# Slienteagle-wyb/tdmpc

Measured on AMD Instinct MI355X. Metric: plan-steps/sec (N=512, H=5, iters=6) at 1/2/4/8 MI355X vs CPU ref, higher is better.
Workload: dtype fp32

## Files before the change

tdmpc_amd/csrc/tdmpc_kernels.hip:

```cpp
#include <hip/hip_runtime.h>
#include <hiprand/hiprand_kernel.h>

#include <math.h>
#include <stdint.h>
#include <stdio.h>
#include <stdlib.h>
#include <string.h>
#include <unistd.h>

#include <algorithm>
#include <atomic>
#include <chrono>
#include <mutex>
#include <type_traits>
#include <vector>

#include "../../include/tdmpc_hip.h"

typedef float floatx16 __attribute__((ext_vector_type(16)));

#define DEVI __device__ __forceinline__

#ifdef TDMPC_STAMPS
__device__ unsigned long long* g_stamps;
// ... 3118 lines not shown
    return a;
}

struct Ctx {
    const tdmpc_dims* d; Layout w; Work k; const float* pw; hipStream_t s;
    int B, N, P, T, H, A, M, Kx;
    int path;
    long eps_env, eps_cem_off, eps_iter, eps_term_off, eps_act_off;
    mutable int split_pend = 0, split_par = 0, split_first = 0;
    mutable float split_disc = 0.f;
    mutable RowMap split_map = {1 << 30, 0, 0};
    mutable int split_rows = 0, split_t = 0;
    int z0c_ready = 0;
    int fold_ok = 0;
    int fold_heads = 0;
    int fold_policy = 0;
};

float* Xt(const Ctx& c, int t) { return c.k.X + (size_t)t * c.k.x_stride; }
const unsigned short* x6p(const Ctx& c, int i) { return (const unsigned short*)(c.pw + c.w.x6[i]); }
enum { CK_STEP = 0, CK_PI = 1, CK_Q = 2 };
int chain_wgs_kind(int kind) {
    static int v[3] = {-2, -2, -2};
    if (v[kind] == -2) {
        static const char* names[3] = {"TDMPC_CHAIN_WGS_STEP", "TDMPC_CHAIN_WGS_PI", "TDMPC_CHAIN_WGS_Q"};
        const char* e = getenv(names[kind]);
        v[kind] = e ? atoi(e) : -1;
    }
    if (v[kind] >= 0) return v[kind];
    return kind == CK_Q ? chain_wgs() / 2 : chain_wgs();
}

bool use_chain(const Ctx& c, int rows, int nprob, int kind) {
    if (c.path == TDMPC_PATH_LAYERED || c.path == TDMPC_PATH_SPLIT || c.path == TDMPC_PATH_SPLIT_X6 || !chain_shape_ok(c.w))
        return false;
    const int th = chain_wgs_kind(kind);
    return c.path != TDMPC_PATH_AUTO || (th > 0 && (rows + 31) / 32 * nprob >= th);
}

int use_x6(const Ctx& c) {
    if (c.w.M != 512) return 0;
    static int en = -1;
    if (en < 0) {
        const char* e = getenv("TDMPC_X6");
        en = e ? atoi(e) : 3;
    }
    if (en == 2) en = 3;
    if (c.path == TDMPC_PATH_CHAIN_X6 || c.path == TDMPC_PATH_WIDE) return en == 1 || en == 3 ? en : 3;
    if (c.path == TDMPC_PATH_SPLIT_X6) return 1;
    return (c.path == TDMPC_PATH_AUTO || c.path == TDMPC_PATH_CHAIN) ? en : 0;
}

int chain_rb(const Ctx& c, int rows, int nprob) {
    if (!chain16_shape_ok(c.w) || c.path == TDMPC_PATH_CHAIN32 || c.path == TDMPC_PATH_CHAIN_X6 ||
        c.path == TDMPC_PATH_WIDE)
        return 32;
    if (c.path == TDMPC_PATH_CHAIN16) return 16;
    return (rows + 31) / 32 * nprob > num_cus() / 2 ? 32 : 16;
}

ChainArgs chain0(const Ctx& c, int rows, RowMap map, int t, int K1, int q1, int nprob) {
    ChainArgs a;
    memset(&a, 0, sizeof a);
    a.rows = rows; a.M = c.M; a.K1 = K1; a.q1 = q1; a.amap = map;
    a.k1_alg = K1 == c.Kx ? c.w.L + c.w.A : c.w.L;
    a.rb = chain_rb(c, rows, nprob);
    a.x6 = a.rb == 32 ? use_x6(c) : (use_x6(c) ? 1 : 0);
    if (a.x6 == 3 && (c.w.Ap / 4 * 32 > 512 || std::max(c.w.Lr, c.w.Ar) > 4 * 4 * 32)) a.x6 = 1;
    a.nw = a.x6 == 3 ? 4 : 8;
    a.hfl = std::max((int)rup(c.Kx, 32), c.M) * a.rb;
    a.X = Xt(c, t); a.x_ts = (long)c.Kx * 32;
    return a;
}
Opnd xop(const Ctx& c, int t, int q0) { return Opnd{Xt(c, t), (long)c.Kx * 32, q0}; }
Outp xout(const Ctx& c, int t, int q0) { return Outp{Xt(c, t), (long)c.Kx * 32, q0}; }
Opnd hop(const float* H, const Ctx& c, int q0) { return Opnd{H, (long)2 * c.M * 32, q0}; }
Outp hout(float* H, const Ctx& c, int q0) { return Outp{H, (long)2 * c.M * 32, q0}; }
Opnd wop(const Ctx& c, size_t off, int K) { return Opnd{c.pw + off, (long)K * 32, 0}; }

bool use_split(const Ctx& c, int rows) {
    const Layout& w = c.w;
    if (w.M != 512 || rows > c.k.split_rows || (size_t)split_lds_floats(w.Kx, w.M) * 4 > 64 * 1024) return false;
    if (c.path == TDMPC_PATH_SPLIT || c.path == TDMPC_PATH_SPLIT_X6) return true;
    if (c.path != TDMPC_PATH_AUTO || (int)rup(w.Kx, 16) > w.M / 2) return false;
    return !use_chain(c, rows, 2, CK_STEP);
}

bool use_split_pi(const Ctx& c, int rows) {
    const Layout& w = c.w;
    if (w.M != 512 || rows > c.k.split_rows || (size_t)split_lds_floats(w.Lp, w.M) * 4 > 64 * 1024) return false;
    if (c.path == TDMPC_PATH_SPLIT || c.path == TDMPC_PATH_SPLIT_X6) return true;
    if (c.path != TDMPC_PATH_AUTO || (int)rup(w.Lp, 16) > w.M / 2) return false;
    return !use_chain(c, rows, 1, CK_PI);
}

int split_finish(const Ctx& c, int t, int rows, RowMap map, const float* zp, const float* rp, float disc, int first,
                 int last) {
    const Layout& w = c.w;
    SplitFinishArgs f;
    memset(&f, 0, sizeof f);
    f.rows = rows; f.amap = map; f.zpart = zp; f.rpart = rp; f.prow = c.k.split_rows;
    f.n3 = w.Lr; f.L = w.L; f.Lp = w.Lp; f.b3d = c.pw + w.b3d; f.b3r = c.pw + w.b3r;
    f.Xo = Xt(c, t + 1); f.x_ts = (long)c.Kx * 32; f.out_q0 = w.Ap / 4;
    f.G = c.k.G; f.rlast = c.k.rlast; f.disc = disc; f.first = first; f.last = last;
    const long nth = (long)rows * (w.Lp / 4 + 1);
    hipLaunchKernelGGL(split_finish_kernel, dim3((unsigned)((nth + 255) / 256)), dim3(256), 0, c.s, f);
    HIPCHK(hipGetLastError());
    return 0;
}

int flush_split(const Ctx& c) {
    if (!c.split_pend) return 0;
    c.split_pend = 0;
    const int par = 1 - c.split_par;
    const size_t zs = (size_t)SPLIT_S * c.k.split_rows * std::max(c.w.Lr, c.w.Ar), rs = (size_t)SPLIT_S * c.k.split_rows;
    return split_finish(c, c.split_t, c.split_rows, c.split_map, c.k.zpart + par * zs, c.k.rpart_s + par * rs,
                        c.split_disc, c.split_first, 0);
}

int z0c_k1c(const Ctx& c) { return (int)rup(c.w.Ap, 16); }
bool z0c_eligible(const Ctx& c) {
    static const int v = [] { const char* e = getenv("TDMPC_Z0C"); return e ? atoi(e) : 1; }();
    return v && z0c_k1c(c) < (int)rup(c.Kx, 16);
}
int z0c_launch(const Ctx& c) {
    hipLaunchKernelGGL(z0c_kernel, dim3(c.B, 2, (c.M + 255) / 256), dim3(256), 0, c.s, c.pw + c.w.w1x, c.pw + c.w.b1x,
                       c.k.z0, c.Kx, c.w.Ap, c.w.Lp, z0c_k1c(c), c.M, c.k.z0c);
    HIPCHK(hipGetLastError());
    return 0;
}

unsigned long long* g_p1_stamps = nullptr;

int wide_g1(const Ctx& c, bool z0c) {
    return (int)rup(z0c ? z0c_k1c(c) : c.Kx, 32) / 32;
}
bool wide_instance(int g1, int nb3, int mode) {
#define WIDE_HAS(G1, NB3, MODE) if (g1 == G1 && nb3 == NB3 && mode == (MODE)) return true;
    WIDE_FOR_EACH(WIDE_HAS)
#undef WIDE_HAS
    return false;
}
bool use_wide(const Ctx& c, int rows, const RowMap& map, bool z0c) {
    static const int en = [] { const char* e = getenv("TDMPC_WIDE"); return e ? atoi(e) : 1; }();
    if (c.w.M != 512 || !use_x6(c) || !num_cus()) return false;
    if (c.path != TDMPC_PATH_AUTO && c.path != TDMPC_PATH_CHAIN && c.path != TDMPC_PATH_WIDE) return false;
    if (c.path != TDMPC_PATH_WIDE && !en) return false;
    if (rows % 16 || map.G % 16 || map.S % 16 || map.O % 16) return false;
    if (z0c && map.G % 128) return false;
    const int g1 = wide_g1(c, z0c), nb3 = (int)rup(c.w.L, 16) / 16, mode = g1 > 5 ? WS_XS : 0;
    if (!wide_instance(g1, nb3, mode) || (c.w.fold && !wide_instance(g1, nb3, mode | WS_OUTH))) return false;
    return c.path == TDMPC_PATH_WIDE || (rows + 127) / 128 * 2 >= num_cus();
}
bool fold_on() {
    static const int v = [] { const char* e = getenv("TDMPC_FOLD"); return e ? atoi(e) : 1; }();
    return v != 0;
}
int launch_wide(const Ctx& c, int t, int rows, RowMap map, float disc, int first, int last, bool z0c, bool fold = false) {
    const Layout& w = c.w;
    const int M = c.M;
    WideArgs a;
    memset(&a, 0, sizeof a);
    auto q6 = [&](int i) { return (const unsigned short*)(c.pw + w.x6q[i]); };
    a.g1s = (int)(rup(c.Kx, 32) / 32);
    const size_t rb1 = (size_t)(M / 16) * a.g1s * 1536;
    const bool fold_in = fold && t >= 1 && !z0c, outh = fold && (!last || c.fold_heads);
    a.p[0].X1 = q6(X6_W1X); a.p[1].X1 = q6(X6_W1X) + rb1;
    a.p[0].X2 = q6(X6_W2D); a.p[1].X2 = q6(X6_W2R);
    a.p[0].b1 = c.pw + w.b1x; a.p[1].b1 = c.pw + w.b1x + M;
    if (fold_in) {
        const unsigned short* xf = (const unsigned short*)(c.pw + w.x6qw);
        a.p[0].X1 = xf; a.p[1].X1 = xf + rb1;
        a.p[0].b1 = c.pw + w.bfw; a.p[1].b1 = c.pw + w.bfw + M;
    }
    a.p[0].b2 = c.pw + w.b2d; a.p[1].b2 = c.pw + w.b2r;
    a.p[1].w3v = c.pw + w.w3r; a.p[1].b3v = c.pw + w.b3r;
    a.X3 = q6(X6_W3D); a.b3 = c.pw + w.b3d; a.nvalid = w.L; a.nstore = w.Lp;
    a.rows = rows; a.nrb = (rows + 127) / 128; a.amap = map;
    a.X = Xt(c, t); a.x_ts = (long)c.Kx * 32;
    a.kq = (z0c ? z0c_k1c(c) : c.Kx) / 4;
    a.Xo = Xt(c, t + 1); a.out_q0 = w.Ap / 4;
    a.G = c.k.G; a.rlast = c.k.rlast; a.disc = disc; a.first = first; a.last = last;
    if (z0c) { a.z0c = c.k.z0c; a.z0_G = map.G; }
    a.stamps = g_p1_stamps;
    const int g1 = wide_g1(c, z0c), nb3 = (int)rup(w.L, 16) / 16;
    const int mode = (g1 > 5 ? WS_XS : 0) | (outh ? WS_OUTH : 0);
    const dim3 grid((unsigned)rup(a.nrb, 4) * 2), block(64 * WS_NW);
    Profiler& pf = g_prof;
    const bool prof = prof_armed() && pf.cfg == 4 + CH_STEP && (pf.rows == 0 || rows == pf.rows) && !z0c;
    if (prof) {
        if (mode) snprintf(pf.kernel, sizeof pf.kernel, "wide_step_kernel<%d, %d, %s%s%s>", g1, nb3,
                           mode & WS_XS ? "XS" : "", mode == (WS_XS | WS_OUTH) ? "|" : "", mode & WS_OUTH ? "OUTH" : "");
        else snprintf(pf.kernel, sizeof pf.kernel, "wide_step_kernel<%d, %d>", g1, nb3);
    }
    HIPCHK(prof_begin(prof, c.s));
    bool done = false;
#define WIDE_LAUNCH(G1, NB3, MODE) \
    if (!done && g1 == G1 && nb3 == NB3 && mode == (MODE)) { \
        hipLaunchKernelGGL((wide_step_kernel<G1, NB3, MODE>), grid, block, (wsm_lds<G1, MODE>()), c.s, a); \
        done = true; \
    }
    WIDE_FOR_EACH(WIDE_LAUNCH)
#undef WIDE_LAUNCH
    if (!done) { snprintf(g_err, sizeof g_err, "wide step: no instance for G1 %d NB3 %d mode %d", g1, nb3, mode); return TDMPC_E_DIMS; }
    HIPCHK(hipGetLastError());
    const double K1 = w.L + w.A;
    HIPCHK(prof_end(prof, c.s, 2.0 * rows * (2 * (K1 * M + (double)M * M) + (outh ? 0.0 : (double)M * w.L) + M)));
    return 0;
}

size_t x6_w1_rows_stride(const Ctx& c) { return (size_t)(c.M / 32) * (rup(c.Kx, 16) / 16) * 1536; }

void step_probs(const Ctx& c, ChainProb (&p)[2], bool x6) {
    const Layout& w = c.w;
    ChainProb& d = p[0];
    d.W1 = c.pw + w.w1x; d.b1 = c.pw + w.b1x; d.W2 = c.pw + w.w2d; d.b2 = c.pw + w.b2d;
    ChainProb& r = p[1];
    r.W1 = c.pw + w.w1x + (size_t)c.M * c.Kx; r.b1 = c.pw + w.b1x + c.M; r.W2 = c.pw + w.w2r; r.b2 = c.pw + w.b2r;
    r.w3v = c.pw + w.w3r;
    if (x6) {
        d.X1 = x6p(c, X6_W1X); r.X1 = d.X1 + x6_w1_rows_stride(c);
        d.X2 = x6p(c, X6_W2D); r.X2 = x6p(c, X6_W2R);
    }
}
void pi_prob(const Ctx& c, ChainProb& p, bool x6) {
    const Layout& w = c.w;
    p.W1 = c.pw + w.wp1; p.b1 = c.pw + w.bp1; p.W2 = c.pw + w.wp2; p.b2 = c.pw + w.bp2;
    if (x6) { p.X1 = x6p(c, X6_WP1); p.X2 = x6p(c, X6_WP2); }
}

int launch_split(const Ctx& c, const SplitArgs& a, int heads, bool x6) {
    const dim3 grid((a.rows + 15) / 16, SPLIT_S, heads);
    const size_t lds = (size_t)split_lds_floats(a.K1, a.M) * 4;
#define SPLIT_LAUNCH(NT, D, X6) \
    if (a.M == 128 * NT && x6 == (X6 != 0)) hipLaunchKernelGGL((split_step_kernel<NT, D, X6>), grid, dim3(512), lds, c.s, a);
    SPLIT_FOR_EACH(SPLIT_LAUNCH)
#undef SPLIT_LAUNCH
    HIPCHK(hipGetLastError());
    return 0;
}


int step_next(const Ctx& c, int t, int rows, RowMap map, float disc, int first, int last, int defer = 0,
              bool nowide = false, bool fold = false) {
    const Layout& w = c.w;
    const int M = c.M;
    int rc;
    if (c.split_pend && (!use_split(c, rows) || rows != c.split_rows || t != c.split_t + 1 ||
                         memcmp(&map, &c.split_map, sizeof map)))
        if ((rc = flush_split(c))) return rc;
    {
        const bool z0c = t == 0 && c.z0c_ready && map.G % 32 == 0;
        if (!nowide && use_wide(c, rows, map, z0c)) {
            if ((rc = flush_split(c))) return rc;
            const RowMap rm = {c.N, map.S, 0}, pm = {c.P, map.S, c.N};
            const int envs = rows / std::max(1, map.G);
            const bool z0c_rm = t == 0 && c.z0c_ready;
            if (c.P > 0 && c.N + c.P == c.T && map.G == c.T && map.S == c.T && map.O == 0 && rows == envs * c.T &&
                use_wide(c, envs * c.N, rm, z0c_rm)) {
                if ((rc = launch_wide(c, t, envs * c.N, rm, disc, first, last, z0c_rm, c.fold_ok))) return rc;
                return step_next(c, t, envs * c.P, pm, disc, first, last, 0, true, c.fold_policy != 0);
            }
            const bool sampled = map.G == c.N && map.S == c.T && map.O == 0;
            return launch_wide(c, t, rows, map, disc, first, last, z0c, c.fold_ok && sampled);
        }
    }
    if (use_chain(c, rows, 2, CK_STEP)) {
        ChainArgs a = chain0(c, rows, map, t, c.Kx, 0, 2);
        step_probs(c, a.p, a.x6 != 0);
        a.p[1].b3v = c.pw + w.b3r;
        a.W3 = c.pw + w.w3d; a.b3 = c.pw + w.b3d; a.n3 = w.Lr; a.nvalid = w.L; a.nstore = w.Lp;
        if (a.x6) a.X3 = x6p(c, X6_W3D);
        a.Xo = Xt(c, t + 1); a.out_q0 = w.Ap / 4;
        a.G = c.k.G; a.rlast = c.k.rlast; a.disc = disc; a.first = first; a.last = last;
        if (t == 0 && c.z0c_ready && map.G % 32 == 0) { a.z0c = c.k.z0c; a.z0_G = map.G; a.k1c = z0c_k1c(c); }
        if (fold) {
            if (a.rb != 32 || !a.x6 || !c.w.fold) {
                snprintf(g_err, sizeof g_err, "folded step: chain_kernel x6 only");
                return TDMPC_E_DIMS;
            }
            if (t >= 1) {
                a.p[0].X1 = (const unsigned short*)(c.pw + w.fw1_x6); a.p[1].X1 = a.p[0].X1 + x6_w1_rows_stride(c);
                a.p[0].b1 = c.pw + w.bfw; a.p[1].b1 = c.pw + w.bfw + M;
            }
            a.outh = 1;
        }
        return launch_chain(CH_STEP, a, 2, c.s);
    }
    if (use_split(c, rows)) {
        const int par = c.split_par;
        const size_t zs = (size_t)SPLIT_S * c.k.split_rows * std::max(w.Lr, w.Ar), rs = (size_t)SPLIT_S * c.k.split_rows;
        SplitArgs a;
        memset(&a, 0, sizeof a);
        a.rows = rows; a.M = M; a.K1 = c.Kx; a.q1 = 0; a.amap = map;
        a.X = Xt(c, t); a.x_ts = (long)c.Kx * 32;
        const bool x6 = use_x6(c) != 0;
        step_probs(c, a.p, x6);
        a.W3 = c.pw + w.w3d; a.n3 = w.Lr;
        if (x6) a.X3 = x6p(c, X6_W3D);
        a.zpart = c.k.zpart + par * zs; a.rpart = c.k.rpart_s + par * rs; a.prow = c.k.split_rows;
        a.b3d = c.pw + w.b3d; a.b3r = c.pw + w.b3r; a.L = w.L; a.Lp = w.Lp; a.zq0 = w.Ap / 4;
        if (c.split_pend) {
            a.zin = c.k.zpart + (1 - par) * zs; a.rin = c.k.rpart_s + (1 - par) * rs;
            a.Xw = Xt(c, t); a.G = c.k.G; a.disc_in = c.split_disc; a.first_in = c.split_first;
        }
        if ((rc = launch_split(c, a, 2, x6))) return rc;
        c.split_pend = 0;
        c.split_par = 1 - par;
        if (defer && !last) {
            c.split_pend = 1; c.split_disc = disc; c.split_first = first;
            c.split_map = map; c.split_rows = rows; c.split_t = t;
            return 0;
        }
        return split_finish(c, t, rows, map, a.zpart, a.rpart, disc, first, last);
    }
    {
        LinArgs a = args0();
        a.M = rows; a.K = c.Kx; a.a_mapped = 1; a.amap = map;
        LinProb& p = a.p[0];
        p.A = xop(c, t, 0); p.W = wop(c, w.w1x, c.Kx); p.bias = c.pw + w.b1x;
        p.C = hout(c.k.H1, c, 0); p.N = p.nvalid = p.nstore = 2 * M; p.epi = EPI_ELU;
        if ((rc = launch_lin(a, 1, 2 * M, 0, PRO_PLAIN, c.s))) return rc;
    }
    {
        LinArgs a = args0();
        a.M = rows; a.K = M;
        LinProb& p0 = a.p[0];
        p0.A = hop(c.k.H1, c, 0); p0.W = wop(c, w.w2d, M); p0.bias = c.pw + w.b2d;
        p0.C = hout(c.k.H2, c, 0); p0.N = p0.nvalid = p0.nstore = M; p0.epi = EPI_ELU;
        LinProb& p1 = a.p[1];
        p1.A = hop(c.k.H1, c, M / 4); p1.W = wop(c, w.w2r, M); p1.bias = c.pw + w.b2r;
        p1.N = p1.nvalid = M; p1.nstore = 0; p1.epi = EPI_ELU_DOT;
        p1.dotw = c.pw + w.w3r; p1.dot_out = c.k.rpart; p1.dot_ld = M / pick_cfg(rows, M, M, 0).bw;
        if ((rc = launch_lin(a, 2, M, 0, PRO_PLAIN, c.s))) return rc;
    }
    {
        LinArgs a = args0();
        a.M = rows; a.K = M; a.c_mapped = 1; a.cmap = map;
        LinProb& p = a.p[0];
        p.A = hop(c.k.H2, c, 0); p.W = wop(c, w.w3d, M); p.bias = c.pw + w.b3d;
        p.C = xout(c, t + 1, w.Ap / 4); p.N = w.L; p.nvalid = w.L; p.nstore = w.Lp; p.epi = EPI_LIN_Z;
        a.rpart = c.k.rpart; a.rpart_nt = M / pick_cfg(rows, M, M, 0).bw; a.b3r = c.pw + w.b3r;
        a.G = c.k.G; a.rlast = c.k.rlast; a.disc = disc; a.first = first; a.last = last;
        if ((rc = launch_lin(a, 1, w.L, 0, PRO_PLAIN, c.s))) return rc;
    }
    return 0;
}

int policy(const Ctx& c, int t, int rows, RowMap map, const float* eps, long eps_env, int eps_G, long eps_off,
           float min_std, float* mu_out = nullptr, bool fold = false) {
    const Layout& w = c.w;
    const int M = c.M;
    int rc;
    if (fold && !(use_chain(c, rows, 1, CK_PI) && use_x6(c))) {
        snprintf(g_err, sizeof g_err, "folded pi: chain x6 kernels only");
        return TDMPC_E_DIMS;
    }
    if (use_chain(c, rows, 1, CK_PI)) {
        ChainArgs a = chain0(c, rows, map, t, w.Lp, w.Ap / 4, 1);
        ChainProb& p = a.p[0];
        pi_prob(c, p, a.x6 != 0);
        a.W3 = c.pw + w.wp3; a.b3 = c.pw + w.bp3; a.n3 = w.Ar; a.nvalid = w.A; a.nstore = w.Ap;
        if (a.x6) a.X3 = x6p(c, X6_WP3);
        if (fold) { p.X1 = (const unsigned short*)(c.pw + w.fpi_x6); p.b1 = c.pw + w.fpi_b; }
        a.Xo = Xt(c, t); a.out_q0 = 0;
        a.eps = eps; a.eps_G = eps_G; a.eps_env = eps_env; a.eps_off = eps_off; a.A = w.A;
        a.min_std = min_std; a.lo = (float)(-1.0 + 1e-6); a.hi = (float)(1.0 - 1e-6);
        a.mu_out = mu_out;
        return launch_chain(CH_PI, a, 1, c.s);
    }
    if (use_split_pi(c, rows)) {
        if ((rc = flush_split(c))) return rc;
        SplitArgs a;
        memset(&a, 0, sizeof a);
        a.rows = rows; a.M = M; a.K1 = w.Lp; a.q1 = w.Ap / 4; a.amap = map;
        a.X = Xt(c, t); a.x_ts = (long)c.Kx * 32;
        const bool x6 = use_x6(c) != 0;
        pi_prob(c, a.p[0], x6);
        a.W3 = c.pw + w.wp3; a.n3 = w.Ar;
        if (x6) a.X3 = x6p(c, X6_WP3);
        a.zpart = c.k.zpart; a.rpart = c.k.rpart_s; a.prow = c.k.split_rows;
        if ((rc = launch_split(c, a, 1, x6))) return rc;
        SplitPiArgs f;
        memset(&f, 0, sizeof f);
        f.rows = rows; f.amap = map; f.part = c.k.zpart; f.prow = c.k.split_rows; f.n3 = w.Ar; f.A = w.A;
        f.Ap = w.Ap; f.b3 = c.pw + w.bp3; f.Xo = Xt(c, t); f.x_ts = (long)c.Kx * 32;
        f.eps = eps; f.eps_G = eps_G; f.eps_env = eps_env; f.eps_off = eps_off; f.min_std = min_std;
        f.lo = (float)(-1.0 + 1e-6); f.hi = (float)(1.0 - 1e-6);
        const long nth = (long)rows * (w.Ap / 4);
        hipLaunchKernelGGL(split_pi_finish_kernel, dim3((unsigned)((nth + 255) / 256)), dim3(256), 0, c.s, f);
        HIPCHK(hipGetLastError());
        return 0;
    }
    {
        LinArgs a = args0();
        a.M = rows; a.K = w.Lp; a.a_mapped = 1; a.amap = map;
        LinProb& p = a.p[0];
        p.A = xop(c, t, w.Ap / 4); p.W = wop(c, w.wp1, w.Lp); p.bias = c.pw + w.bp1;
        p.C = hout(c.k.H1, c, 0); p.N = p.nvalid = p.nstore = M; p.epi = EPI_ELU;
        if ((rc = launch_lin(a, 1, M, 0, PRO_PLAIN, c.s))) return rc;
    }
    {
        LinArgs a = args0();
        a.M = rows; a.K = M;
        LinProb& p = a.p[0];
        p.A = hop(c.k.H1, c, 0); p.W = wop(c, w.wp2, M); p.bias = c.pw + w.bp2;
        p.C = hout(c.k.H2, c, 0); p.N = p.nvalid = p.nstore = M; p.epi = EPI_ELU;
        if ((rc = launch_lin(a, 1, M, 0, PRO_PLAIN, c.s))) return rc;
    }
    {
        LinArgs a = args0();
        a.M = rows; a.K = M; a.c_mapped = 1; a.cmap = map;
        LinProb& p = a.p[0];
        p.A = hop(c.k.H2, c, 0); p.W = wop(c, w.wp3, M); p.bias = c.pw + w.bp3;
        p.C = xout(c, t, 0); p.N = w.A; p.nvalid = w.A; p.nstore = w.Ap; p.epi = EPI_PI;
        a.eps = eps; a.eps_G = eps_G; a.eps_env = eps_env; a.eps_off = eps_off; a.A = w.A;
        a.min_std = min_std;
// ... 1039 lines not shown
```

tdmpc_amd/csrc/wide_ring.inc:

```

constexpr int WS_NW = 8;
constexpr int WS_AHEAD = 2;
constexpr int WS_FRAG = 3072;
constexpr int WS_SLOT = WS_NW * WS_FRAG;
template <int G1> constexpr int ws_xbytes() { return WS_NW * G1 * 2048; }
template <int G1> constexpr int ws_ns() {
    return (160 * 1024 - ws_xbytes<G1>()) / WS_SLOT < 6 ? (160 * 1024 - ws_xbytes<G1>()) / WS_SLOT : 6;
}
template <int G1> constexpr size_t ws_lds() { return (size_t)ws_ns<G1>() * WS_SLOT + ws_xbytes<G1>(); }

DEVI void ws_glds(const void* gsrc, unsigned voff, unsigned lds) {
    unsigned keep;
    asm volatile("s_mov_b32 %0, m0\n\ts_mov_b32 m0, %2\n\ts_nop 0\n\t"
                 "global_load_lds_dwordx4 %1, %3\n\ts_mov_b32 m0, %0"
                 : "=&s"(keep)
                 : "v"(voff), "s"(lds), "s"(gsrc)
                 : "memory");
}
DEVI void w2_glds(const void* gsrc, unsigned voff, unsigned lds) {
    const unsigned long long g = (unsigned long long)gsrc;
    const unsigned glo = __builtin_amdgcn_readfirstlane((unsigned)g), ghi = __builtin_amdgcn_readfirstlane((unsigned)(g >> 32));
    const unsigned long long gs = ((unsigned long long)ghi << 32) | glo;
    const unsigned ls = __builtin_amdgcn_readfirstlane(lds);
    unsigned keep;
    asm volatile("s_nop 4\n\ts_mov_b32 %0, m0\n\ts_mov_b32 m0, %2\n\ts_nop 0\n\t"
                 "global_load_lds_dwordx4 %1, %3\n\ts_mov_b32 m0, %0"
                 : "=&s"(keep)
                 : "v"(voff), "s"(ls), "s"(gs)
                 : "memory");
}

DEVI void w2_x6(floatx4& acc, const uint4& u0, const uint4& u1, const uint4& u2, const X6U& b) {
    const bf16x8_t w0 = as_bf16x8(u0), w1 = as_bf16x8(u1), w2 = as_bf16x8(u2);
    const bf16x8_t bh = as_bf16x8(b.h), bm = as_bf16x8(b.m), bl = as_bf16x8(b.l);
    acc = __builtin_amdgcn_mfma_f32_16x16x32_bf16(w1, bm, acc, 0, 0, 0);
    acc = __builtin_amdgcn_mfma_f32_16x16x32_bf16(w2, bh, acc, 0, 0, 0);
    acc = __builtin_amdgcn_mfma_f32_16x16x32_bf16(w0, bl, acc, 0, 0, 0);
    acc = __builtin_amdgcn_mfma_f32_16x16x32_bf16(w1, bh, acc, 0, 0, 0);
    acc = __builtin_amdgcn_mfma_f32_16x16x32_bf16(w0, bm, acc, 0, 0, 0);
    acc = __builtin_amdgcn_mfma_f32_16x16x32_bf16(w0, bh, acc, 0, 0, 0);
}

typedef X6U WSX;
DEVI WSX ws_opnd(const float4& a0, const float4& a1, bool fin) {
#ifdef WS_DIAG_NOSPLIT
    (void)fin;
    X6U b;
    b.h = b.m = b.l = *(const uint4*)&a0;
    return b;
#else
    X6U b;
    if (fin) b = w2_split8_fin(a0, a1);
    else b = w2_split8(a0, a1);
    return b;
#endif
}
DEVI void ws_prod(floatx4& acc, const uint4& u0, const uint4& u1, const uint4& u2, const WSX& b) { w2_x6(acc, u0, u1, u2, b); }

typedef const __attribute__((address_space(4))) float w2cf;

template <int NS, int SLOT, int VM, void (*DMA)(const void*, unsigned, unsigned)>
struct WRing {
    char* ring;
    unsigned lds, voff;
    int lane, wave, k;
    uint4 fc[WS_AHEAD][3];
#ifdef WS_STAMPS
    unsigned long long* st = nullptr;
#endif
    DEVI WRing(char* base, int lane_, int wave_)
        : ring(base), lds((unsigned)(size_t)(__attribute__((address_space(3))) char*)base), voff(lane_ * 16),
          lane(lane_), wave(wave_), k(0) {}

    DEVI void issue(int kk, const unsigned short* src) const {
        const unsigned dst = lds + (unsigned)((kk % NS) * SLOT + wave * WS_FRAG);
#pragma unroll
        for (int p = 0; p < 3; ++p) DMA(src + p * 512, voff, dst + p * 1024);
    }
    template <class After>
    DEVI const char* sync(const unsigned short* nsrc, After after) {
#ifdef WS_STAMPS
        if (st && k < 256) st[2 * k] = __builtin_amdgcn_s_memtime();
#endif
        asm volatile("s_waitcnt vmcnt(%0)\n\ts_barrier" :: "n"(VM) : "memory");
#ifdef WS_STAMPS
        if (st && k < 256) st[2 * k + 1] = __builtin_amdgcn_s_memtime();
#endif
        const char* sl = ring + (k % NS) * SLOT + lane * 16;
        issue(k + NS - 1, nsrc);
        after(k + NS - 1);
        ++k;
        return sl;
    }
    DEVI const char* sync(const unsigned short* nsrc) { return sync(nsrc, [](int) {}); }

    static DEVI void rd(uint4 (&f)[3], const char* p) {
        f[0] = *(const uint4*)p;
        f[1] = *(const uint4*)(p + 1024);
        f[2] = *(const uint4*)(p + 2048);
    }
    DEVI void prime() {
#pragma unroll
        for (int d = 0; d < WS_AHEAD; ++d) rd(fc[d], ring + d * WS_FRAG + lane * 16);
    }
    DEVI void frag(const char* sl, int i, uint4& w0, uint4& w1, uint4& w2) {
        w0 = fc[0][0];
        w1 = fc[0][1];
        w2 = fc[0][2];
#pragma unroll
        for (int d = 0; d + 1 < WS_AHEAD; ++d)
#pragma unroll
            for (int p = 0; p < 3; ++p) fc[d][p] = fc[d + 1][p];
        rd(fc[WS_AHEAD - 1], i + WS_AHEAD <= WS_NW - 1 ? sl + (i + WS_AHEAD) * WS_FRAG
                                                       : ring + (k % NS) * SLOT + (i + WS_AHEAD - WS_NW) * WS_FRAG + lane * 16);
        __builtin_amdgcn_sched_barrier(0);
    }
};

template <int G1>
DEVI const unsigned short* wr_src(const unsigned short* const& X1, const int& g1s, const unsigned short* const& X2, int wave,
                                  int sc, int j) {
    if (j < G1) return X1 + ((size_t)(8 * sc + wave) * g1s + j) * 1536;
    const int s2 = j - G1, co = s2 >> 3, st = s2 & 7;
    return X2 + ((size_t)(8 * (st & 3) + wave) * 16 + 2 * (2 * sc + co) + (st >> 2)) * 1536;
}
template <int G1, int NS, class Src, class Tail>
DEVI const unsigned short* wr_next(Src src, Tail tail, int sc, int j) {
    const int jt = j + NS - 1;
    if (jt < G1 + 16) return src(sc, jt);
    return sc < 3 ? src(sc + 1, jt - (G1 + 16)) : tail(jt - (G1 + 16));
}
template <int NB>
DEVI const unsigned short* wr_l3_src(const unsigned short* const& X3, int l, int wave) {
    const int f3 = 8 * l + wave;
    return X3 + ((size_t)(f3 % NB) * 16 + f3 / NB) * 1536;
}

template <int G1>
DEVI bool wr_xtile(p1f4* sx, const float* const& X, const long& x_ts, int xr0, int n, int q, const int& q0, const int& kq,
                   bool live) {
    const float* xp = X + (size_t)(xr0 >> 5) * x_ts + (size_t)q0 * 128 + ((xr0 & 31) + n) * 4;
    const p1f4 zero4 = {0.f, 0.f, 0.f, 0.f};
    float xsum = 0.f;
#pragma unroll
    for (int g = 0; g < G1; ++g) {
        const int qa = 8 * g + q, qb = qa + 4;
        const p1f4 va = live && qa < kq ? *(const p1f4*)(xp + (size_t)qa * 128) : zero4;
        const p1f4 vb = live && qb < kq ? *(const p1f4*)(xp + (size_t)qb * 128) : zero4;
        sx[(2 * g) * 64] = va;
        sx[(2 * g + 1) * 64] = vb;
        xsum += ((va[0] + va[1]) + (va[2] + va[3])) + ((vb[0] + vb[1]) + (vb[2] + vb[3]));
    }
    return ws_wave_finite(xsum);
}

DEVI void wr_lane_ep(unsigned voff, int& n_ep, int& q_ep) {
    int l16 = (int)voff;
    asm volatile("" : "+v"(l16));
    n_ep = (l16 >> 4) & 15;
    q_ep = (l16 >> 8) & 3;
}
DEVI float4 wr_h2t(const floatx4 (&acc)[32], const float* sb2, int t, int q) {
    const float4 bv = *(const float4*)(sb2 + 16 * t + 4 * q);
    return make_float4(elu_f(acc[t][0] + bv.x), elu_f(acc[t][1] + bv.y), elu_f(acc[t][2] + bv.z), elu_f(acc[t][3] + bv.w));
}

DEVI void x6_put(unsigned short* d, size_t blk, int lane, int j, __bf16 hi, __bf16 md, __bf16 lo) {
    d[(blk * 3 + 0) * 512 + lane * 8 + j] = __builtin_bit_cast(unsigned short, hi);
    d[(blk * 3 + 1) * 512 + lane * 8 + j] = __builtin_bit_cast(unsigned short, md);
    d[(blk * 3 + 2) * 512 + lane * 8 + j] = __builtin_bit_cast(unsigned short, lo);
}
DEVI void x6q_put(unsigned short* d, int G, int r, int kk, float x) {
    __bf16 hi, md, lo;
    split3(x, hi, md, lo);
    const int nb = r / 16, g = kk / 32, k2 = kk % 32;
    const int lane = (r % 16) + 16 * ((k2 % 16) / 4), j = 4 * (k2 / 16) + (k2 % 4);
    x6_put(d, (size_t)nb * G + g, lane, j, hi, md, lo);
}
```

tdmpc_amd/csrc/wide_step.inc:

```

enum { WS_XS = 1, WS_OUTH = 2 };
constexpr int WS_XAREA = WS_NW * 2048;
template <int G1, int MODE> constexpr int wsm_slot() { return (MODE & WS_XS) ? WS_SLOT + WS_XAREA : WS_SLOT; }
template <int G1, int MODE> constexpr int wsm_ns() {
    return (MODE & WS_XS) ? (160 * 1024 / wsm_slot<G1, MODE>() < 6 ? 160 * 1024 / wsm_slot<G1, MODE>() : 6) : ws_ns<G1>();
}
template <int G1, int MODE> constexpr size_t wsm_lds() {
    return (MODE & WS_XS) ? (size_t)wsm_ns<G1, MODE>() * wsm_slot<G1, MODE>() : ws_lds<G1>();
}
template <int G1, int MODE> constexpr int wsm_bias() {
    return (MODE & WS_XS) ? (wsm_ns<G1, MODE>() - 1) * wsm_slot<G1, MODE>() + WS_SLOT : ws_ns<G1>() * WS_SLOT;
}

#if (defined(WS_DIAG_NODMA) || defined(WS_DIAG_NOSPLIT)) && !defined(TDMPC_VARIANT)
#error "WS_DIAG_* diagnostics produce wrong results: build them only as a named variant (tdmpc_amd.build --variant)"
#endif

struct WideHead {
    const unsigned short* X1;
    const unsigned short* X2;
    const float* b1; const float* b2;
    const float* w3v; const float* b3v;
};

struct WideArgs {
    WideHead p[2];
    const unsigned short* X3; const float* b3; int nvalid, nstore;
    int rows, nrb;
    RowMap amap;
    const float* X; long x_ts;
    int kq;
    int g1s;
    float* Xo; int out_q0;
    float* G; float* rlast; float disc; int first, last;
    const float* z0c; int z0_G;
    unsigned long long* stamps;
};

template <bool SGPR>
DEVI void ws_dma(const void* gsrc, unsigned voff, unsigned lds) {
#ifndef WS_DIAG_NODMA
    if constexpr (SGPR) ws_glds(gsrc, voff, lds);
    else w2_glds(gsrc, voff, lds);
#else
    (void)gsrc; (void)voff; (void)lds;
#endif
}

template <int G1, int NB3, int MODE>
__global__ void __launch_bounds__(64 * WS_NW) __attribute__((amdgpu_waves_per_eu(2, 2)))
wide_step_kernel(const WideArgs a) {
    constexpr bool XS = (MODE & WS_XS) != 0, OUTH = (MODE & WS_OUTH) != 0;
    constexpr int WS_NS = wsm_ns<G1, MODE>();
    constexpr int SLOT = wsm_slot<G1, MODE>();
    constexpr int VM = XS ? 3 : 3 * (WS_NS - 3);
    constexpr int SPC2 = G1 + 16;
    constexpr int NP3 = NB3 > 8 ? NB3 / 8 : 1;
    constexpr int TAIL = OUTH ? 0 : (NB3 > 8 ? 16 * NP3 : 2 * NB3);
    static_assert(NB3 <= 8 || NB3 % 8 == 0, "layer-3 passes of 8 tiles");
    static_assert(WS_NS >= 3 && WS_NS - 1 < SPC2, "ring depth");
    static_assert(wsm_lds<G1, MODE>() <= 160 * 1024, "wide step LDS");
    static_assert(XS ? WS_XAREA >= 6 * 1024 : ws_xbytes<G1>() >= 6 * 1024, "bias area");
    extern __shared__ __attribute__((aligned(16))) char wsm[];
    const int tid = threadIdx.x, lane = tid & 63, n = lane & 15, q = lane >> 4;
    const int wave = __builtin_amdgcn_readfirstlane(tid >> 6);
    const int bid = blockIdx.x;
    const int head = (bid & 7) >> 2;
    const int rb = (bid >> 3) * 4 + (bid & 3);
    if (rb >= a.nrb) return;
    const WideHead& P = a.p[head];
    p1f4* sx = (p1f4*)(wsm + WS_NS * WS_SLOT) + wave * (G1 * 2 * 64) + lane;
    const float* sb2 = (const float*)(wsm + wsm_bias<G1, MODE>());
    const float* sw3 = sb2 + 512;
    const float* sb3 = sw3 + 512;
    const int m0 = rb * 128 + wave * 16;
    const bool live = m0 < a.rows;
    const int xr0 = live ? map_row(a.amap, m0) : 0;

    WRing<WS_NS, SLOT, VM, ws_dma<MODE == 0 && NB3 <= 8>> R(wsm, lane, wave);
    auto src_main2 = [&](int sc, int j) __attribute__((always_inline)) { return wr_src<G1>(P.X1, a.g1s, P.X2, wave, sc, j); };
    auto src_tail = [&](int l) __attribute__((always_inline)) -> const unsigned short* {
        if (!OUTH && head == 0 && l < TAIL) {
            if constexpr (NB3 > 8) {
                return a.X3 + ((size_t)(8 * (l >> 4) + wave) * 16 + (l & 15)) * 1536;
            } else {
                return wr_l3_src<NB3>(a.X3, l, wave);
            }
        }
        return P.X2;
    };
    auto src_next2 = [&](int sc, int j) __attribute__((always_inline)) { return wr_next<G1, WS_NS>(src_main2, src_tail, sc, j); };
    const float* xrow = a.X + (size_t)(xr0 >> 5) * a.x_ts;
    const unsigned xlo = (unsigned)(((xr0 & 31) + n) * 16);
    auto issue_x = [&](int kk, int xg) __attribute__((always_inline)) {
        if constexpr (XS) {
            if (xg >= 0) {
                const unsigned xdst = R.lds + (unsigned)((kk % WS_NS) * SLOT + WS_SLOT + wave * 2048);
                const int qa = min(8 * xg + q, a.kq - 1), qb = min(8 * xg + 4 + q, a.kq - 1);
                ws_dma<false>(xrow, xlo + (unsigned)qa * 512u, xdst);
                ws_dma<false>(xrow, xlo + (unsigned)qb * 512u, xdst + 1024);
            }
        }
    };
    auto xg_next2 = [&](int sc, int j) __attribute__((always_inline)) -> int {
        const int jt = j + WS_NS - 1;
        if (jt < SPC2) return jt < G1 ? jt : -1;
        return sc < 3 && jt - SPC2 < G1 ? jt - SPC2 : -1;
    };
#pragma unroll
    for (int k = 0; k < WS_NS - 1; ++k) {
        R.issue(k, src_main2(0, k));
        issue_x(k, k < G1 ? k : -1);
    }
    bool xfin = true;
    if constexpr (!XS) xfin = wr_xtile<G1>(sx, a.X, a.x_ts, xr0, n, q, 0, a.kq, live);
    const float* b1src = a.z0c ? a.z0c + ((size_t)(rb * 128 < a.rows ? rb * 128 / a.z0_G : 0) * 2 + head) * 512
                               : P.b1;
    float g_old = 0.f;
    if (head == 1 && q == 0 && live && !a.first) g_old = a.G[xr0 + n];
    asm volatile("" :: "v"(g_old));
    asm volatile("s_waitcnt vmcnt(0) lgkmcnt(0)\n\ts_barrier" ::: "memory");
#ifdef WS_STAMPS
    if (a.stamps && (bid == 0 || bid == 4) && lane == 0) R.st = a.stamps + (bid ? 4096 : 0) + wave * 512;
#endif
    R.prime();

    floatx4 acc[32];
#pragma unroll
    for (int j = 0; j < 32; ++j) acc[j] = floatx4{0.f, 0.f, 0.f, 0.f};

#pragma unroll 1
    for (int sc = 0; sc < 4; ++sc) {
        auto sync = [&](int j, bool tail_bias) __attribute__((always_inline)) {
            return R.sync(src_next2(sc, j), [&](int kk) __attribute__((always_inline)) {
                issue_x(kk, xg_next2(sc, j));
                if (tail_bias && wave < 4) {
                    const float* bsrc = wave < 2 ? P.b2 + 256 * wave : head == 1 ? P.w3v + 256 * (wave - 2) : a.b3 + 256 * (wave - 2);
                    const unsigned bdst = R.lds + (unsigned)wsm_bias<G1, MODE>() + (unsigned)(wave < 2 || head == 1 ? wave : wave + 2) * 1024;
                    if (wave < 2 || head == 1 || (!OUTH && (wave - 2) * 256 < 16 * NB3))
                        ws_dma<MODE == 0 && NB3 <= 8>(bsrc, R.voff, bdst);
                }
            });
        };
        floatx4 a1[8];
#pragma unroll
        for (int b = 0; b < 8; ++b) a1[b] = floatx4{0.f, 0.f, 0.f, 0.f};
        constexpr int UG1 = XS ? 1 : G1;
#pragma unroll UG1
        for (int g = 0; g < G1; ++g) {
            const char* sl = sync(g, false);
            p1f4 x0, x1;
            bool fin = xfin;
            if constexpr (XS) {
                const p1f4 zero4 = {0.f, 0.f, 0.f, 0.f};
                const p1f4* xs = (const p1f4*)(sl + WS_SLOT + wave * 2048);
                x0 = xs[0];
                x1 = xs[64];
                if (!live || 8 * g + q >= a.kq) x0 = zero4;
                if (!live || 8 * g + 4 + q >= a.kq) x1 = zero4;
                fin = ws_wave_finite(((x0[0] + x0[1]) + (x0[2] + x0[3])) + ((x1[0] + x1[1]) + (x1[2] + x1[3])));
            } else {
                x0 = sx[(2 * g) * 64];
                x1 = sx[(2 * g + 1) * 64];
            }
            const WSX xb = ws_opnd(make_float4(x0[0], x0[1], x0[2], x0[3]), make_float4(x1[0], x1[1], x1[2], x1[3]), fin);
#pragma unroll
            for (int b = 0; b < 8; ++b) {
                uint4 w0, w1, w2;
                R.frag(sl, b, w0, w1, w2);
                ws_prod(a1[b], w0, w1, w2, xb);
            }
        }
#pragma unroll
        for (int co = 0; co < 2; ++co) {
            const int c = 2 * sc + co;
#pragma unroll
            for (int b = 0; b < 4; ++b) {
                const w2cf* bv = (const w2cf*)b1src + 64 * c + 16 * b;
#pragma unroll
                for (int i = 0; i < 4; ++i)
                    a1[4 * co + b][i] = elu_f(a1[4 * co + b][i] + (q == 0 ? bv[i] : q == 1 ? bv[4 + i] : q == 2 ? bv[8 + i] : bv[12 + i]));
            }
            const floatx4* t = a1 + 4 * co;
            const bool hfin = ws_wave_finite(ws_sum8(make_float4(t[0][0], t[0][1], t[0][2], t[0][3]),
                                                     make_float4(t[1][0], t[1][1], t[1][2], t[1][3])) +
                                             ws_sum8(make_float4(t[2][0], t[2][1], t[2][2], t[2][3]),
                                                     make_float4(t[3][0], t[3][1], t[3][2], t[3][3])));
#pragma unroll
            for (int s2 = 0; s2 < 2; ++s2) {
                const floatx4& t0 = t[2 * s2];
                const floatx4& t1 = t[2 * s2 + 1];
                const WSX xb = ws_opnd(make_float4(t0[0], t0[1], t0[2], t0[3]), make_float4(t1[0], t1[1], t1[2], t1[3]), hfin);
#pragma unroll
                for (int jq = 0; jq < 4; ++jq) {
                    const int j2 = G1 + 8 * co + 4 * s2 + jq;
                    const char* sl = sync(j2, sc == 3 && co == 0 && s2 == 0 && jq == 0);
#pragma unroll
                    for (int jj = 0; jj < 8; ++jj) {
                        uint4 w0, w1, w2;
                        R.frag(sl, jj, w0, w1, w2);
                        ws_prod(acc[8 * jq + jj], w0, w1, w2, xb);
                    }
                }
            }
        }
    }
    int n_ep, q_ep;
    wr_lane_ep(R.voff, n_ep, q_ep);

    if (head == 0 && OUTH) {
        asm volatile("s_waitcnt vmcnt(0)" ::: "memory");
        if (live) {
            const int xr = xr0 + n_ep;
            float* xo = a.Xo + (size_t)(xr >> 5) * a.x_ts + (xr & 31) * 4;
#pragma unroll
            for (int t = 0; t < 32; ++t) *(float4*)(xo + (size_t)(a.out_q0 + 4 * t + q_ep) * 128) = wr_h2t(acc, sb2, t, q);
        }
    } else if (head == 0 && NB3 > 8) {
        floatx4 a3[8];
        const char* sl = nullptr;
#pragma unroll 1
        for (int p = 0; p < NP3; ++p) {
#pragma unroll
            for (int j = 0; j < 8; ++j) a3[j] = floatx4{0.f, 0.f, 0.f, 0.f};
            auto l3group = [&](int g) __attribute__((always_inline)) {
                const float4 ha = wr_h2t(acc, sb2, 2 * g, q), hb = wr_h2t(acc, sb2, 2 * g + 1, q);
                const WSX xb = ws_opnd(ha, hb, ws_wave_finite(ws_sum8(ha, hb)));
                sl = R.sync(src_tail(16 * p + g + WS_NS - 1));
#pragma unroll
                for (int jj = 0; jj < 8; ++jj) {
                    uint4 w0, w1, w2;
                    R.frag(sl, jj, w0, w1, w2);
                    ws_prod(a3[jj], w0, w1, w2, xb);
                }
            };
#pragma unroll
            for (int g = 0; g < 8; ++g) l3group(g);
#pragma unroll
            for (int g = 8; g < 16; ++g) l3group(g);
            if (live) {
                const int xr = xr0 + n_ep;
                float* xo = a.Xo + (size_t)(xr >> 5) * a.x_ts + (xr & 31) * 4;
#pragma unroll
                for (int jj = 0; jj < 8; ++jj) {
                    const int cq = 4 * (8 * p + jj) + q_ep, col = 4 * cq;
                    if (col < a.nstore) {
                        const float4 bv = *(const float4*)(sb3 + col);
                        float o[4] = {a3[jj][0] + bv.x, a3[jj][1] + bv.y, a3[jj][2] + bv.z, a3[jj][3] + bv.w};
#pragma unroll
                        for (int e = 0; e < 4; ++e)
                            if (col + e >= a.nvalid) o[e] = 0.f;
                        *(float4*)(xo + (size_t)(a.out_q0 + cq) * 128) = make_float4(o[0], o[1], o[2], o[3]);
                    }
                }
            }
        }
        asm volatile("s_waitcnt vmcnt(0)" ::: "memory");
    } else if (head == 0) {
        floatx4 a3[NB3 > 8 ? 1 : NB3];
        constexpr int NB = NB3 > 8 ? 1 : NB3;
#pragma unroll
        for (int j = 0; j < NB; ++j) a3[j] = floatx4{0.f, 0.f, 0.f, 0.f};
        WSX xb;
        const char* sl = nullptr;
        auto l3group = [&](int g) __attribute__((always_inline)) {
            const float4 ha = wr_h2t(acc, sb2, 2 * g, q), hb = wr_h2t(acc, sb2, 2 * g + 1, q);
            xb = ws_opnd(ha, hb, ws_wave_finite(ws_sum8(ha, hb)));
#pragma unroll
            for (int jj = 0; jj < NB; ++jj) {
                const int f = g * NB + jj;
                if (f % WS_NW == 0) sl = R.sync(src_tail(f / WS_NW + WS_NS - 1));
                uint4 w0, w1, w2;
                R.frag(sl, f % WS_NW, w0, w1, w2);
                ws_prod(a3[jj], w0, w1, w2, xb);
            }
        };
#pragma unroll
        for (int g = 0; g < 8; ++g) l3group(g);
#pragma unroll
        for (int g = 8; g < 16; ++g) l3group(g);
        asm volatile("s_waitcnt vmcnt(0)" ::: "memory");
        if (live) {
            const int xr = xr0 + n_ep;
            float* xo = a.Xo + (size_t)(xr >> 5) * a.x_ts + (xr & 31) * 4;
#pragma unroll
            for (int jj = 0; jj < NB; ++jj) {
                const int cq = 4 * jj + q_ep, col = 4 * cq;
                if (col < a.nstore) {
                    const float4 bv = *(const float4*)(sb3 + col);
                    float o[4] = {a3[jj][0] + bv.x, a3[jj][1] + bv.y, a3[jj][2] + bv.z, a3[jj][3] + bv.w};
#pragma unroll
                    for (int e = 0; e < 4; ++e)
                        if (col + e >= a.nvalid) o[e] = 0.f;
                    *(float4*)(xo + (size_t)(a.out_q0 + cq) * 128) = make_float4(o[0], o[1], o[2], o[3]);
                }
            }
        }
    } else {
        float s = 0.f;
#pragma unroll
        for (int t = 0; t < 32; ++t) {
            const float4 v = wr_h2t(acc, sb2, t, q);
            const float4 wv = *(const float4*)(sw3 + 16 * t + 4 * q_ep);
            s += (v.x * wv.x + v.y * wv.y) + (v.z * wv.z + v.w * wv.w);
        }
        s += __shfl_xor(s, 16);
        s += __shfl_xor(s, 32);
        asm volatile("s_waitcnt vmcnt(0)" ::: "memory");
        if (live && q_ep == 0) {
            const int xr = xr0 + n_ep;
            const float o = s + P.b3v[0];
            const float dr = fmul(a.disc, o);
            a.G[xr] = a.first ? dr : fadd(g_old, dr);
            if (a.last) a.rlast[xr] = o;
        }
    }
}

#define WIDE_FOR_EACH(X) X(1, 7, 0) X(2, 7, 0) X(4, 7, 0) X(5, 7, 0) X(1, 4, 0) X(2, 4, 0) X(3, 4, 0) \
    X(1, 32, 0) X(1, 32, WS_OUTH) X(17, 32, WS_XS) X(17, 32, WS_XS | WS_OUTH)
```

Measured before the change: 6221.

## Add loader-wave variant of wide step kernel with 64-row blocks

Adds a WS_LD mode to the wide step kernel. Four of the eight waves become dedicated DMA producers that fill the LDS weight ring, and the other four compute on 64-row blocks instead of 128-row blocks. Consumer waves only barrier and no longer issue loads, so weight streaming is meant to overlap with the MFMA work and more blocks exist to fill the CUs when row counts are small. The host picks this variant for sampled and policy rows when it is allowed and when the 64-row grid covers the CUs. The cost is half the compute waves per block and more complex synchronisation, with restricted instance coverage.

After: 6252 (median of 6 runs). No clear change (+0.5%).

```diff
diff --git a/tdmpc_amd/csrc/tdmpc_kernels.hip b/tdmpc_amd/csrc/tdmpc_kernels.hip
--- a/tdmpc_amd/csrc/tdmpc_kernels.hip
+++ b/tdmpc_amd/csrc/tdmpc_kernels.hip
@@ -3294,11 +3294,22 @@
     if (!wide_instance(g1, nb3, mode) || (c.w.fold && !wide_instance(g1, nb3, mode | WS_OUTH))) return false;
     return c.path == TDMPC_PATH_WIDE || (rows + 127) / 128 * 2 >= num_cus();
 }
+int wide64_mode() { const char* e = getenv("TDMPC_WIDE64"); return e ? atoi(e) : 1; }
+bool use_wide64(const Ctx& c, int rows, const RowMap& map, bool z0c, bool policy) {
+    const int en = wide64_mode();
+    if (en <= 0 || (!policy && en < 2) || c.w.fold) return false;
+    if (rows % 64 || map.G % 16 || map.S % 16 || map.O % 16) return false;
+    if (z0c && map.G % 64) return false;
+    const int g1 = wide_g1(c, z0c), nb3 = (int)rup(c.w.L, 16) / 16;
+    if (g1 > 5 || !wide_instance(g1, nb3, WS_LD) || !wide_instance(wide_g1(c, false), nb3, WS_LD)) return false;
+    return en >= 2 || rows / 64 * 2 >= num_cus();
+}
 bool fold_on() {
     static const int v = [] { const char* e = getenv("TDMPC_FOLD"); return e ? atoi(e) : 1; }();
     return v != 0;
 }
-int launch_wide(const Ctx& c, int t, int rows, RowMap map, float disc, int first, int last, bool z0c, bool fold = false) {
+int launch_wide(const Ctx& c, int t, int rows, RowMap map, float disc, int first, int last, bool z0c, bool fold = false,
+                bool ld = false) {
     const Layout& w = c.w;
     const int M = c.M;
     WideArgs a;
@@ -3318,7 +3329,7 @@
     a.p[0].b2 = c.pw + w.b2d; a.p[1].b2 = c.pw + w.b2r;
     a.p[1].w3v = c.pw + w.w3r; a.p[1].b3v = c.pw + w.b3r;
     a.X3 = q6(X6_W3D); a.b3 = c.pw + w.b3d; a.nvalid = w.L; a.nstore = w.Lp;
-    a.rows = rows; a.nrb = (rows + 127) / 128; a.amap = map;
+    a.rows = rows; a.nrb = ld ? (rows + 63) / 64 : (rows + 127) / 128; a.amap = map;
     a.X = Xt(c, t); a.x_ts = (long)c.Kx * 32;
     a.kq = (z0c ? z0c_k1c(c) : c.Kx) / 4;
     a.Xo = Xt(c, t + 1); a.out_q0 = w.Ap / 4;
@@ -3326,12 +3337,13 @@
     if (z0c) { a.z0c = c.k.z0c; a.z0_G = map.G; }
     a.stamps = g_p1_stamps;
     const int g1 = wide_g1(c, z0c), nb3 = (int)rup(w.L, 16) / 16;
-    const int mode = (g1 > 5 ? WS_XS : 0) | (outh ? WS_OUTH : 0);
+    const int mode = (g1 > 5 ? WS_XS : 0) | (outh ? WS_OUTH : 0) | (ld ? WS_LD : 0);
     const dim3 grid((unsigned)rup(a.nrb, 4) * 2), block(64 * WS_NW);
     Profiler& pf = g_prof;
     const bool prof = prof_armed() && pf.cfg == 4 + CH_STEP && (pf.rows == 0 || rows == pf.rows) && !z0c;
     if (prof) {
-        if (mode) snprintf(pf.kernel, sizeof pf.kernel, "wide_step_kernel<%d, %d, %s%s%s>", g1, nb3,
+        if (mode == WS_LD) snprintf(pf.kernel, sizeof pf.kernel, "wide_step_kernel<%d, %d, LD>", g1, nb3);
+        else if (mode) snprintf(pf.kernel, sizeof pf.kernel, "wide_step_kernel<%d, %d, %s%s%s>", g1, nb3,
                            mode & WS_XS ? "XS" : "", mode == (WS_XS | WS_OUTH) ? "|" : "", mode & WS_OUTH ? "OUTH" : "");
         else snprintf(pf.kernel, sizeof pf.kernel, "wide_step_kernel<%d, %d>", g1, nb3);
     }
@@ -3400,11 +3412,17 @@
             const bool z0c_rm = t == 0 && c.z0c_ready;
             if (c.P > 0 && c.N + c.P == c.T && map.G == c.T && map.S == c.T && map.O == 0 && rows == envs * c.T &&
                 use_wide(c, envs * c.N, rm, z0c_rm)) {
-                if ((rc = launch_wide(c, t, envs * c.N, rm, disc, first, last, z0c_rm, c.fold_ok))) return rc;
+                if ((rc = launch_wide(c, t, envs * c.N, rm, disc, first, last, z0c_rm, c.fold_ok,
+                                      use_wide64(c, envs * c.N, rm, z0c_rm, false))))
+                    return rc;
+                const bool z0c_pm = t == 0 && c.z0c_ready && pm.G % 32 == 0;
+                if (!c.fold_policy && use_wide64(c, envs * c.P, pm, z0c_pm, true))
+                    return launch_wide(c, t, envs * c.P, pm, disc, first, last, z0c_pm, false, true);
                 return step_next(c, t, envs * c.P, pm, disc, first, last, 0, true, c.fold_policy != 0);
             }
             const bool sampled = map.G == c.N && map.S == c.T && map.O == 0;
-            return launch_wide(c, t, rows, map, disc, first, last, z0c, c.fold_ok && sampled);
+            return launch_wide(c, t, rows, map, disc, first, last, z0c, c.fold_ok && sampled,
+                               sampled && use_wide64(c, rows, map, z0c, false));
         }
     }
     if (use_chain(c, rows, 2, CK_STEP)) {
diff --git a/tdmpc_amd/csrc/wide_ring.inc b/tdmpc_amd/csrc/wide_ring.inc
--- a/tdmpc_amd/csrc/wide_ring.inc
+++ b/tdmpc_amd/csrc/wide_ring.inc
@@ -59,7 +59,7 @@
 
 typedef const __attribute__((address_space(4))) float w2cf;
 
-template <int NS, int SLOT, int VM, void (*DMA)(const void*, unsigned, unsigned)>
+template <int NS, int SLOT, int VM, void (*DMA)(const void*, unsigned, unsigned), bool LD = false>
 struct WRing {
     char* ring;
     unsigned lds, voff;
@@ -82,15 +82,36 @@
 #ifdef WS_STAMPS
         if (st && k < 256) st[2 * k] = __builtin_amdgcn_s_memtime();
 #endif
-        asm volatile("s_waitcnt vmcnt(%0)\n\ts_barrier" :: "n"(VM) : "memory");
+        if constexpr (LD) asm volatile("s_barrier" ::: "memory");
+        else asm volatile("s_waitcnt vmcnt(%0)\n\ts_barrier" :: "n"(VM) : "memory");
 #ifdef WS_STAMPS
         if (st && k < 256) st[2 * k + 1] = __builtin_amdgcn_s_memtime();
 #endif
         const char* sl = ring + (k % NS) * SLOT + lane * 16;
-        issue(k + NS - 1, nsrc);
+        if constexpr (!LD) {
+            issue(k + NS - 1, nsrc);
+            after(k + NS - 1);
+        }
+        ++k;
+        return sl;
+    }
+    template <class Src>
+    DEVI void issue2(int kk, int lw, Src src) const {
+#pragma unroll
+        for (int e = 0; e < 2; ++e) {
+            const int f = 2 * lw + e;
+            const unsigned short* s = src(f);
+            const unsigned dst = lds + (unsigned)((kk % NS) * SLOT + f * WS_FRAG);
+#pragma unroll
+            for (int p = 0; p < 3; ++p) DMA(s + p * 512, voff, dst + p * 1024);
+        }
+    }
+    template <class Src, class After>
+    DEVI void produce(int lw, Src src, After after) {
+        asm volatile("s_waitcnt vmcnt(%0)\n\ts_barrier" :: "n"(VM) : "memory");
+        issue2(k + NS - 1, lw, src);
         after(k + NS - 1);
         ++k;
-        return sl;
     }
     DEVI const char* sync(const unsigned short* nsrc) { return sync(nsrc, [](int) {}); }
 
diff --git a/tdmpc_amd/csrc/wide_step.inc b/tdmpc_amd/csrc/wide_step.inc
--- a/tdmpc_amd/csrc/wide_step.inc
+++ b/tdmpc_amd/csrc/wide_step.inc
@@ -1,5 +1,5 @@
 
-enum { WS_XS = 1, WS_OUTH = 2 };
+enum { WS_XS = 1, WS_OUTH = 2, WS_LD = 4 };
 constexpr int WS_XAREA = WS_NW * 2048;
 template <int G1, int MODE> constexpr int wsm_slot() { return (MODE & WS_XS) ? WS_SLOT + WS_XAREA : WS_SLOT; }
 template <int G1, int MODE> constexpr int wsm_ns() {
@@ -50,10 +50,12 @@
 template <int G1, int NB3, int MODE>
 __global__ void __launch_bounds__(64 * WS_NW) __attribute__((amdgpu_waves_per_eu(2, 2)))
 wide_step_kernel(const WideArgs a) {
-    constexpr bool XS = (MODE & WS_XS) != 0, OUTH = (MODE & WS_OUTH) != 0;
+    constexpr bool XS = (MODE & WS_XS) != 0, OUTH = (MODE & WS_OUTH) != 0, LD = (MODE & WS_LD) != 0;
+    static_assert(!LD || MODE == WS_LD, "loader waves: not with the latent-512 modes");
+    constexpr int RB = LD ? 64 : 128;
     constexpr int WS_NS = wsm_ns<G1, MODE>();
     constexpr int SLOT = wsm_slot<G1, MODE>();
-    constexpr int VM = XS ? 3 : 3 * (WS_NS - 3);
+    constexpr int VM = XS ? 3 : (LD ? 6 : 3) * (WS_NS - 3);
     constexpr int SPC2 = G1 + 16;
     constexpr int NP3 = NB3 > 8 ? NB3 / 8 : 1;
     constexpr int TAIL = OUTH ? 0 : (NB3 > 8 ? 16 * NP3 : 2 * NB3);
@@ -73,11 +75,11 @@
     const float* sb2 = (const float*)(wsm + wsm_bias<G1, MODE>());
     const float* sw3 = sb2 + 512;
     const float* sb3 = sw3 + 512;
-    const int m0 = rb * 128 + wave * 16;
+    const int m0 = rb * RB + (LD ? wave & 3 : wave) * 16;
     const bool live = m0 < a.rows;
     const int xr0 = live ? map_row(a.amap, m0) : 0;
 
-    WRing<WS_NS, SLOT, VM, ws_dma<MODE == 0 && NB3 <= 8>> R(wsm, lane, wave);
+    WRing<WS_NS, SLOT, VM, ws_dma<MODE == 0 && NB3 <= 8>, LD> R(wsm, lane, wave);
     auto src_main2 = [&](int sc, int j) __attribute__((always_inline)) { return wr_src<G1>(P.X1, a.g1s, P.X2, wave, sc, j); };
     auto src_tail = [&](int l) __attribute__((always_inline)) -> const unsigned short* {
         if (!OUTH && head == 0 && l < TAIL) {
@@ -107,14 +109,52 @@
         if (jt < SPC2) return jt < G1 ? jt : -1;
         return sc < 3 && jt - SPC2 < G1 ? jt - SPC2 : -1;
     };
-#pragma unroll
-    for (int k = 0; k < WS_NS - 1; ++k) {
-        R.issue(k, src_main2(0, k));
-        issue_x(k, k < G1 ? k : -1);
+    if constexpr (LD) {
+        if (wave >= 4) {
+            const int lw = wave - 4;
+            auto main_w = [&](int w) __attribute__((always_inline)) {
+                return [&, w](int sc, int j) __attribute__((always_inline)) { return wr_src<G1>(P.X1, a.g1s, P.X2, w, sc, j); };
+            };
+            auto tail_w = [&](int w) __attribute__((always_inline)) {
+                return [&, w](int l) __attribute__((always_inline)) -> const unsigned short* {
+                    return head == 0 && l < TAIL ? wr_l3_src<NB3>(a.X3, l, w) : P.X2;
+                };
+            };
+#pragma unroll
+            for (int k = 0; k < WS_NS - 1; ++k)
+                R.issue2(k, lw, [&](int w) __attribute__((always_inline)) { return main_w(w)(0, k); });
+            asm volatile("s_waitcnt vmcnt(0) lgkmcnt(0)\n\ts_barrier" ::: "memory");
+#pragma unroll 1
+            for (int sc = 0; sc < 4; ++sc) {
+#pragma unroll
+                for (int j = 0; j < SPC2; ++j)
+                    R.produce(lw, [&](int w) __attribute__((always_inline)) { return wr_next<G1, WS_NS>(main_w(w), tail_w(w), sc, j); },
+                              [&](int) __attribute__((always_inline)) {
+                                  if (sc == 3 && j == G1) {
+                                      const float* bsrc = lw < 2 ? P.b2 + 256 * lw : head == 1 ? P.w3v + 256 * (lw - 2) : a.b3 + 256 * (lw - 2);
+                                      const unsigned bdst = R.lds + (unsigned)wsm_bias<G1, MODE>() + (unsigned)(lw < 2 || head == 1 ? lw : lw + 2) * 1024;
+                                      if (lw < 2 || head == 1 || (lw - 2) * 256 < 16 * NB3) ws_dma<false>(bsrc, R.voff, bdst);
+                                  }
+                              });
+            }
+            if (head == 0) {
+#pragma unroll 1
+                for (int l = 0; l < TAIL; ++l)
+                    R.produce(lw, [&](int w) __attribute__((always_inline)) { return tail_w(w)(l + WS_NS - 1); }, [](int) {});
+            }
+            asm volatile("s_waitcnt vmcnt(0)" ::: "memory");
+            return;
+        }
+    } else {
+#pragma unroll
+        for (int k = 0; k < WS_NS - 1; ++k) {
+            R.issue(k, src_main2(0, k));
+            issue_x(k, k < G1 ? k : -1);
+        }
     }
     bool xfin = true;
     if constexpr (!XS) xfin = wr_xtile<G1>(sx, a.X, a.x_ts, xr0, n, q, 0, a.kq, live);
-    const float* b1src = a.z0c ? a.z0c + ((size_t)(rb * 128 < a.rows ? rb * 128 / a.z0_G : 0) * 2 + head) * 512
+    const float* b1src = a.z0c ? a.z0c + ((size_t)(rb * RB < a.rows ? rb * RB / a.z0_G : 0) * 2 + head) * 512
                                : P.b1;
     float g_old = 0.f;
     if (head == 1 && q == 0 && live && !a.first) g_old = a.G[xr0 + n];
@@ -318,4 +358,5 @@
 }
 
 #define WIDE_FOR_EACH(X) X(1, 7, 0) X(2, 7, 0) X(4, 7, 0) X(5, 7, 0) X(1, 4, 0) X(2, 4, 0) X(3, 4, 0) \
-    X(1, 32, 0) X(1, 32, WS_OUTH) X(17, 32, WS_XS) X(17, 32, WS_XS | WS_OUTH)
+    X(1, 32, 0) X(1, 32, WS_OUTH) X(17, 32, WS_XS) X(17, 32, WS_XS | WS_OUTH) \
+    X(1, 7, WS_LD) X(4, 7, WS_LD) X(1, 4, WS_LD) X(2, 4, WS_LD)
```
